# vitasoftAI/ImageRetrievalResearch

Hardware: AMD Instinct MI355X
Metric: images/sec embed + queries/sec top-k@100k-gallery, EffNet-B3a 224^2 (higher is better)
Workload: dtype bf16

## Files before the change

### imageretrievalresearch_amd/_lib.py

```python
from __future__ import annotations

import ctypes as C
import os

_HERE = os.path.dirname(os.path.abspath(__file__))
LIB_PATH = os.environ.get("MI355_LIB_PATH") or os.path.join(_HERE, "libmi355_retrieval.so")

c_f32p = C.POINTER(C.c_float)
c_i64p = C.POINTER(C.c_int64)
vp = C.c_void_p


class GemmExArgs(C.Structure):
    _fields_ = [("A", vp), ("lda", C.c_int), ("W", vp), ("ldw", C.c_int), ("bias", vp),
                ("res", vp), ("ldr", C.c_int), ("res_n", C.c_int),
                ("gate", vp), ("gate_ld", C.c_int), ("rows_per_img", C.c_int), ("a_relu6", C.c_int),
                ("out", vp), ("ldo", C.c_int), ("out_f32", C.c_int),
                ("M", C.c_int), ("N", C.c_int), ("K", C.c_int), ("act", C.c_int),
                ("M_sel", C.c_int64), ("splitk_ws", vp), ("splitk_ws_bytes", C.c_size_t),
                ("ln_stats", vp), ("ln_colsum", vp)]


class RankFilter(C.Structure):
    _fields_ = [("query_labels", vp), ("gallery_labels", vp), ("label_mode", C.c_int), ("exclude", vp)]
# ... 51 lines not shown
    "mi355_model_num_tensors": (C.c_int, [vp]),
    "mi355_model_tensor_info": (C.c_int, [vp, C.c_int, C.POINTER(C.c_char_p), C.POINTER(C.c_int),
                                          C.POINTER(C.c_int64), C.POINTER(C.c_int)]),
    "mi355_model_feature_dim": (C.c_int, [vp]),
    "mi355_model_num_classes": (C.c_int, [vp]),
    "mi355_model_set_tensor": (C.c_int, [vp, C.c_char_p, vp, C.c_int64]),
    "mi355_model_pack": (C.c_int, [vp, vp]),
    "mi355_model_forward_features": (C.c_int, [vp, vp, C.c_int, C.c_int, C.c_int, vp, vp, vp]),
    "mi355_model_forward": (C.c_int, [vp, vp, C.c_int, C.c_int, C.c_int, vp, vp, vp]),
    "mi355_model_forward_u8": (C.c_int, [vp, vp, C.c_int, C.c_int, C.c_int, C.c_int, C.POINTER(C.c_float), C.POINTER(C.c_float),
                                         vp, C.c_int, vp, vp, vp]),
    "mi355_model_enable_taps": (C.c_int, [vp, C.c_int]),
    "mi355_model_read_tap": (C.c_int, [vp, C.c_char_p, vp, C.c_int64, C.POINTER(C.c_int64), vp]),
    "mi355_model_run_between_taps": (C.c_int, [vp, C.c_char_p, C.c_char_p, vp, C.c_int, C.c_int, C.c_int, C.c_int, vp]),
    "mi355_model_traffic": (C.c_int, [vp, C.c_int, C.c_int, C.c_int, C.POINTER(C.c_double),
                                      C.POINTER(C.c_double), C.POINTER(C.c_double)]),
    "mi355_model_traffic_kinds": (C.c_int, [vp, C.c_int, C.c_int, C.c_int, C.POINTER(C.c_double),
                                            C.POINTER(C.c_double), C.c_int]),
    "mi355_model_set_option": (C.c_int, [vp, C.c_char_p, C.c_int64]),
    "mi355_model_profile_read": (C.c_int, [vp, C.POINTER(C.c_double), C.POINTER(C.c_int64), C.c_int]),
    "mi355_model_profile_ops": (C.c_int, [vp, C.c_int, C.c_int, C.c_int, C.c_int, C.POINTER(C.c_double),
                                          C.POINTER(C.c_double), C.POINTER(C.c_int), C.c_char_p, C.c_int]),
    "mi355_model_block_stamps": (C.c_int, [vp, C.POINTER(C.c_double), C.c_int]),
    "mi355_pool_linear": (C.c_int, [vp, C.c_int, C.c_int, C.c_int, vp, vp, C.c_int, vp, vp, vp]),
    "mi355_gemm_bf16": (C.c_int, [vp, vp, vp, vp, C.c_int, C.c_int, C.c_int, C.c_int, C.c_int, vp]),
    "mi355_gemm_bf16_ex": (C.c_int, [vp, C.POINTER(C.c_int), vp]),
    "mi355_window_attention": (C.c_int, [vp, vp, vp, C.c_int, C.c_int, C.c_int, C.c_int, C.c_int, vp]),
    "mi355_square_pad_normalize": (C.c_int, [vp, C.c_int, C.c_int, C.c_int, C.POINTER(C.c_float), C.POINTER(C.c_float), vp, vp]),
    "mi355_conv_input_silu": (C.c_int, [vp, vp, C.c_int, C.c_int, C.c_int, vp, vp]),
    "mi355_resize_bilinear_u8": (C.c_int, [vp, C.c_int, C.c_int, vp, C.c_int, C.c_int, vp, vp]),
    "mi355_resize_batch_workspace_bytes": (C.c_size_t, [vp, C.c_int, C.c_int, C.c_int, C.c_int]),
    "mi355_resize_batch_u8": (C.c_int, [vp, C.c_int64, vp, vp, C.c_int, C.c_int, C.c_int, C.c_int, C.c_int, vp, vp, C.c_size_t,
                                        vp]),
    "mi355_model_forward_images_workspace_bytes": (C.c_size_t, [vp, C.c_int, C.c_int, C.c_int]),
    "mi355_model_forward_images": (C.c_int, [vp, vp, C.c_int64, vp, vp, C.c_int, C.c_int, C.c_int, C.c_int, C.POINTER(C.c_float),
                                             C.POINTER(C.c_float), vp, C.c_int, vp, vp, vp, C.c_size_t, vp]),
    "mi355_score_boost": (C.c_int, [vp, C.c_int64, C.c_float, C.c_float, C.c_float, C.c_int, vp, vp]),
}

_lib = None


class MI355Error(RuntimeError):
    """A libmi355_retrieval call returned nonzero; the message is mi355_last_error()."""


# ... 33 lines not shown
```

### imageretrievalresearch_amd/csrc/mbconv_block.hip

```cpp
#include "ops.h"

namespace mi355 {

typedef __bf16 bf16x8 __attribute__((ext_vector_type(8)));
typedef float f32x4 __attribute__((ext_vector_type(4)));
typedef unsigned u32x4 __attribute__((ext_vector_type(4)));
typedef unsigned u32x2 __attribute__((ext_vector_type(2)));

constexpr int MB_THREADS = 512;
constexpr int MB_WAVES = MB_THREADS / 64;
constexpr int MB_MAX_RD = 192;
constexpr int MB_MC = MB_WAVES * 16;

__device__ __forceinline__ float mb_lo(unsigned u) { return __uint_as_float(u << 16); }
__device__ __forceinline__ float mb_hi(unsigned u) { return __uint_as_float(u & 0xffff0000u); }

__device__ __forceinline__ void mb_lds_barrier() {
    asm volatile("s_waitcnt lgkmcnt(0)" ::: "memory");
    __builtin_amdgcn_s_barrier();
    asm volatile("" ::: "memory");
}

__host__ __device__ static inline int mb_proj_ntw(int NTp, int MTp, int NTW) {
    int best = 1, best_busy = 0;
// ... 12 lines not shown
    const int ntw = mb_proj_ntw(NTp, MTp, 3);
    if (wi != 14) return ntw;
    const int nwn = (NTp + ntw - 1) / ntw;
    int msplit = nwn <= MB_WAVES ? MB_WAVES / nwn : 1;
    if (msplit > MTp) msplit = MTp;
    if (nwn <= MB_WAVES && (MTp + msplit - 1) / msplit <= mwp) return ntw;
    return 4;
}

template <int KS> struct MbTaps {
    static constexpr int KK = KS * KS;
    static constexpr int NV = (KS / 2) * KS;
    static constexpr int NH = (KS + 1) / 2;
    static constexpr int NP = NV + NH;
    __host__ __device__ static constexpr bool vertical(int tp) { return tp < NV; }
    __host__ __device__ static constexpr int tap_a(int tp) {
        return tp < NV ? (tp / KS) * 2 * KS + tp % KS : (KS - 1) * KS + (tp - NV) * 2;
    }
    __host__ __device__ static constexpr int tap_b(int tp) {
        return tp < NV ? tap_a(tp) + KS : ((tp - NV) * 2 + 1 < KS ? tap_a(tp) + 1 : -1);
    }
};

template <int KS, int S, int WI, int MW, int MH, int NTW, int MWP, int KST, int A_IT, int ACT_E, int ACT_D>
__global__ __launch_bounds__(MB_THREADS) void k_mbconv_block(const BlockArgs a) {
    using TP = MbTaps<KS>;
    constexpr int MC = MB_MC;
    constexpr int PAD = KS / 2;
    constexpr int NP = TP::NP;
    constexpr int EW = WI + 2 * PAD;
    constexpr int WO = (WI + 2 * PAD - KS) / S + 1;
    constexpr int TR = WO <= 8 ? 2 : 1;
    constexpr int RP = (TR == 2 && S == 1) ? ((EW + 7) & ~7) : EW;
    static_assert(WO <= 16, "depthwise tile geometry");
    constexpr bool PROJ_WHOLE = WI == 7 && NTW == 2;
    constexpr int KC = WI == 7 ? 256 : 128;
    constexpr int ALD = KC + 16;
    extern __shared__ __attribute__((aligned(16))) unsigned char mb_smem[];

    const int tid = threadIdx.x, lane = tid & 63;
    const int wave = __builtin_amdgcn_readfirstlane(tid >> 6);
    const int fr = lane & 15, fq = lane >> 4, fk = fq * 8;
    const int b = blockIdx.x;
    const int P = a.H * a.W, MT = (P + 15) >> 4, XLD = a.XLD;
    const int EH = a.H + 2 * PAD;
    const int EP = (EH + (TR == 2 ? S : 0)) * RP + 8;
    const int Pout = a.Ho * a.Wo;
    const int MTo = TR == 2 ? (a.Ho + 1) >> 1 : a.Ho;
    const int midp = (a.mid + 15) & ~15;

    bf16_t* Xs = reinterpret_cast<bf16_t*>(mb_smem);
    size_t off = ((size_t)MT * 16 * XLD * 2 + 64 + 15) & ~(size_t)15;
    float* pool = reinterpret_cast<float*>(mb_smem + off);
    off += (size_t)((a.mid + 255) & ~255) * 4;
    float* rvec = reinterpret_cast<float*>(mb_smem + off);
    off += MB_MAX_RD * 4;
    unsigned char* R = mb_smem + off;
    bf16_t* Es = reinterpret_cast<bf16_t*>(R) + (size_t)wave * EP * 16;

    const bool stamping = a.stamps != nullptr;
    unsigned t_acc[8] = {0, 0, 0, 0, 0, 0, 0, 0};
    unsigned t_last = 0;
    if (stamping) t_last = (unsigned)__builtin_readcyclecounter();
    auto tick = [&](int i) {
        if (stamping) { const unsigned t = (unsigned)__builtin_readcyclecounter(); t_acc[i] += t - t_last; t_last = t; }
    };

    const int nslabs = (a.mid + MC - 1) / MC;
    const int rb0 = (a.norot & 1) ? 0 : b, rb1 = (a.norot & 2) ? 0 : b, rb2 = (a.norot & 4) ? 0 : b, rb3 = (a.norot & 8) ? 0 : b;
    auto slab_of = [&](int ci) { return (ci + rb0) % nslabs; };

    u32x4 wq[KST];
    f32x4 be_reg;
    auto w_prefetch_slab = [&](int cbase) {
        const int n = min(cbase + wave * 16 + fr, midp - 1);
#pragma unroll
        for (int h = 0; h < KST; ++h) wq[h] = *reinterpret_cast<const u32x4*>(a.We + (n * a.Kp + fk + h * 32));
        be_reg = *reinterpret_cast<const f32x4*>(a.be + min(cbase + wave * 16 + fq * 4, midp - 4));
        __builtin_amdgcn_sched_barrier(0);
    };
    unsigned short wd_raw[NP], wd_nxt[NP];
    f32x4 bd_reg, bd_nxt;
    auto wd_fetch = [&](int cbase) {
        const int ch = min(cbase + wave * 16 + fr, a.mid - 1);
#pragma unroll
        for (int tp = 0; tp < NP; ++tp) {
            const int ta = TP::tap_a(tp), tb = TP::tap_b(tp) < 0 ? TP::tap_a(tp) : TP::tap_b(tp);
            const int t = (lane & 32) ? tb : ta;
            wd_nxt[tp] = a.Wd[t * a.mid + ch];
        }
        bd_nxt = *reinterpret_cast<const f32x4*>(a.bd + min(cbase + wave * 16 + fq * 4, a.mid - 4));
        __builtin_amdgcn_sched_barrier(0);
// ... 22 lines not shown
            if (id0 == tid) {
                bf16_t* Eall = reinterpret_cast<bf16_t*>(R);
                for (int id = tid; id < MB_WAVES * EP * 2; id += MB_THREADS)
                    *reinterpret_cast<u32x4*>(&Eall[id * 8]) = (u32x4){0u, 0u, 0u, 0u};
                if (tid < 4) *reinterpret_cast<u32x4*>(&Xs[MT * 16 * XLD + tid * 8]) = (u32x4){0u, 0u, 0u, 0u};
            }
#pragma unroll
            for (int u = 0; u < U; ++u)
                if (dst[u] >= 0) *reinterpret_cast<u32x4*>(&Xs[dst[u]]) = v[u];
        }
    }
    mb_lds_barrier();
    tick(0);

    bf16_t* Db = a.D + (size_t)b * Pout * a.mid;

    const int e_cv = (fq & 1) * 8 + ((fq >> 1) ? RP * 16 : 0);
    const int e_ch = (fq & 1) * 8 + ((fq >> 1) ? 16 : 0);
    const int t_row = TR == 2 ? (fr >> 3) : 0, t_col = TR == 2 ? (fr & 7) : fr;
    const int e_lane = (t_row * S * RP + t_col * S) * 16;
    constexpr int E_TILE = TR * S * RP * 16;
    const bool col_ok = t_col < WO;

    const int abl = a.variant;
    bool prev_active = false;
    for (int ci = 0; ci < nslabs; ++ci) {
        const int cbase = slab_of(ci) * MC;
        const int ch0 = cbase + wave * 16;
        const bool active = ch0 < a.mid;
        {
            constexpr int MTO_SQ = TR == 2 ? (WO + 1) / 2 : WO;
            if (ci > 0 && prev_active && MTo == MTO_SQ) {
                if constexpr (MTO_SQ >= 14) asm volatile("s_waitcnt vmcnt(14)" ::: "memory");
                else if constexpr (MTO_SQ >= 4) asm volatile("s_waitcnt vmcnt(4)" ::: "memory");
                else asm volatile("s_waitcnt vmcnt(1)" ::: "memory");
            } else {
                asm volatile("s_waitcnt vmcnt(0)" ::: "memory");
            }
#pragma unroll
            for (int h = 0; h < KST; ++h) asm volatile("" : "+v"(wq[h]));
            asm volatile("" : "+v"(be_reg));
            asm volatile("" : "+v"(bd_nxt));
#pragma unroll
            for (int tp = 0; tp < NP; ++tp) { asm volatile("" : "+v"(wd_nxt[tp])); wd_raw[tp] = wd_nxt[tp]; }
            bd_reg = bd_nxt;
        }
        tick(1);
// ... 468 lines not shown
#pragma unroll
                    for (int j = 0; j < NTW; ++j) {
                        const int n = (wn * ntw + j) * 16 + fq * 4;
                        if (j < ntw && n < a.Cout) {
                            float v[4] = {acc[j][i].x, acc[j][i].y, acc[j][i].z, acc[j][i].w};
                            if (a.has_res && n < a.res_n) {
                                v[0] += mb_lo(rr[j][i].x); v[1] += mb_hi(rr[j][i].x); v[2] += mb_lo(rr[j][i].y); v[3] += mb_hi(rr[j][i].y);
                            }
                            u32x2 o;
                            o.x = pack2bf(v[0], v[1]);
                            o.y = pack2bf(v[2], v[3]);
                            *reinterpret_cast<u32x2*>(Yb + (m * a.Cout + n)) = o;
                        }
                    }
                }
            }
        }
    }
    tick(7);
    if (stamping && tid == 0) {
        long long* o = a.stamps + (size_t)b * 16;
#pragma unroll
        for (int i = 0; i < 8; ++i) o[i] = (long long)t_acc[i];
    }
}

struct MbGeom { int wi, mw, mh, ntw, mwp, a_it; };
static bool mb_geom(int H, int W, MbGeom* g) {
    if (W == 7 && H * W <= 64) { *g = {7, 4, 1, 3, 4, 4}; return true; }
    if (W == 14 && H * W <= 208) { *g = {14, 7, 2, 3, 7, 7}; return true; }
    return false;
}
#define MB_INSTANCES(X)                                                                                              \
    X(3, 1, 14, 3, 3, ACT_SILU) X(5, 1, 14, 3, 3, ACT_SILU) X(5, 1, 14, 5, 3, ACT_SILU) X(5, 2, 14, 5, 2, ACT_SILU)     \
    X(5, 1, 7, 8, 2, ACT_SILU) X(3, 1, 7, 8, 3, ACT_SILU) X(3, 1, 7, 12, 3, ACT_SILU)                                 \
    X(3, 1, 14, 4, 2, ACT_NONE) X(3, 1, 14, 4, 3, ACT_NONE) X(3, 1, 14, 5, 3, ACT_NONE) X(3, 1, 14, 6, 3, ACT_NONE)   \
    X(3, 1, 7, 7, 2, ACT_NONE) X(3, 1, 7, 8, 2, ACT_NONE) X(3, 1, 7, 8, 3, ACT_NONE) X(3, 1, 7, 9, 3, ACT_NONE)       \
    X(3, 1, 7, 10, 3, ACT_NONE) X(3, 1, 7, 11, 3, ACT_NONE) X(3, 1, 14, 6, 4, ACT_NONE)
static bool mb_instance_ok(int k, int stride, int wi, int kst, int ntw, int act_d) {
#define X(KS, S, WI, KST, NTW, AD) if (k == KS && stride == S && wi == WI && kst == KST && ntw == NTW && act_d == AD) return true;
    MB_INSTANCES(X)
#undef X
    return false;
}

static int mb_pick_kcs(const BlockArgs& a) {
// ... 68 lines not shown
    return mb_pick_xld(a, k, g) != 0;
}

template <int KS, int S, int WI, int MW, int MH, int NTW, int MWP, int KST, int A_IT, int ACT_E, int ACT_D>
static int launch_mb(BlockArgs a, int B, hipStream_t st) {
    MbGeom g;
    mb_geom(a.H, a.W, &g);
    a.XLD = mb_pick_xld(a, KS, g);
    a.KCS = mb_pick_kcs(a);
    const size_t lds = mb_lds_bytes_xld(a, KS, a.XLD, g);
    static bool attr_done[64] = {false};
    int dev = 0;
    MI355_CHECK_HIP(hipGetDevice(&dev));
    if (dev >= 0 && dev < 64 && !attr_done[dev]) {
        MI355_CHECK_HIP(hipFuncSetAttribute((const void*)k_mbconv_block<KS, S, WI, MW, MH, NTW, MWP, KST, A_IT, ACT_E, ACT_D>,
                                            hipFuncAttributeMaxDynamicSharedMemorySize, 160 * 1024));
        attr_done[dev] = true;
    }
    hipLaunchKernelGGL((k_mbconv_block<KS, S, WI, MW, MH, NTW, MWP, KST, A_IT, ACT_E, ACT_D>), dim3(B), dim3(MB_THREADS), lds, st, a);
    MI355_LAUNCH_CHECK();
    return OK;
}

int launch_mbconv_block(const BlockArgs& a, int B, int k, int stride, hipStream_t st) {
    MI355_REQUIRE(mbconv_block_supported(a.H, a.W, a.Cin, a.mid, a.Cout, k, stride, a.rd, a.act_e, a.act_d), "mbconv_block: unsupported shape");
    const int Pout = a.Ho * a.Wo;
    MbGeom gg;
    mb_geom(a.H, a.W, &gg);
    const int ntw = mb_pick_ntw((a.Cout + 15) / 16, (Pout + 15) / 16, gg.wi, gg.mwp);
    const int kst = a.Kp / 32;
#define X(KS, S, WI, KST, NTW, AD)                                                                  \
    if (k == KS && stride == S && a.W == WI && kst == KST && ntw == NTW && a.act_d == AD)           \
        return launch_mb<KS, S, WI, (WI == 7 ? 4 : 7), (WI == 7 ? 1 : 2), NTW, (WI == 7 ? 4 : 7), KST, (WI == 7 ? 4 : 7), ACT_SILU, AD>(a, B, st);
    MB_INSTANCES(X)
#undef X
    set_error("mbconv_block: no instance for k=%d s=%d W=%d Kp=%d ntw=%d", k, stride, a.W, a.Kp, ntw);
    return ERR_UNSUPPORTED;
}

}
```

### imageretrievalresearch_amd/csrc/model.hip

```cpp
#include "model_exec.h"
#include "../../include/mi355_retrieval.h"

#include <string.h>

#include <algorithm>

namespace mi355 {

int pack_gemm(Packer& pk, Op& op) {
    const TensorSpec* w = pk.get(op.w_name);
    if (!w) return ERR_STATE;
    const int N = op.cout_real, K = op.cin_real;
    MI355_REQUIRE(w->numel() == (int64_t)N * K, "pack: %s has %lld elements, expected %d x %d", op.w_name.c_str(),
                  (long long)w->numel(), N, K);
    std::vector<float> scale, shift;
    if (!pk.bn_fold(op.bn_name, op.bn_eps, N, scale, shift)) return ERR_STATE;
    if (!op.bias_name.empty()) {
        const TensorSpec* b = pk.get(op.bias_name);
        if (!b) return ERR_STATE;
        for (int i = 0; i < N; ++i) shift[i] = b->data[i] * scale[i] + shift[i];
    }
    const int Np = (op.cout + 15) & ~15, Kp = (op.cin + 31) & ~31;
    op.w_off = pk.alloc((size_t)Np * Kp * 2);
    op.b_off = pk.alloc((size_t)Np * 4);
// ... 318 lines not shown
    if (g.out != SLOT_E || d.in != SLOT_E || d.out != SLOT_D || p.in != SLOT_D || !p.use_gate || !d.pool) return false;
    if (g.use_gate || g.res != SLOT_NONE || g.a_relu6 || !g.tap.empty() || !d.tap.empty()) return false;
    if (p.act != ACT_NONE || (p.res != SLOT_NONE && p.res != g.in)) return false;
    if (p.res != SLOT_NONE && p.res_channels && ((p.res_channels + 7) & ~7) != g.cin) return false;
    return mbconv_block_supported(h, w, g.cin, g.cout, p.cout, d.k, d.stride, s.rd, g.act, d.act);
}

static int stamp_ptr(ExecCtx& cx, size_t oi, long long** out) {
    mi355_model* m = cx.m;
    *out = nullptr;
    if (!m->block_stamps) return OK;
    const size_t need = m->def.ops.size() * (size_t)cx.B * 16 * sizeof(long long);
    if (m->stamp_bytes < need) {
        if (m->stamp_buf) MI355_CHECK_HIP(hipFree(m->stamp_buf));
        MI355_CHECK_HIP(hipMalloc((void**)&m->stamp_buf, need));
        m->stamp_bytes = need;
    }
    m->stamp_B = cx.B;
    *out = m->stamp_buf + (oi * (size_t)cx.B + cx.b0) * 16;
    MI355_CHECK_HIP(hipMemsetAsync(*out, 0, (size_t)cx.nb * 16 * sizeof(long long), cx.st));
    return OK;
}

static int exec_block(ExecCtx& cx, size_t oi) {
    mi355_model* m = cx.m;
    SlotState* S = m->slots;
    const Op& g = m->def.ops[oi];
    const Op& d = m->def.ops[oi + 1];
    const Op& s = m->def.ops[oi + 2];
    const Op& p = m->def.ops[oi + 3];
    BlockArgs a{};
    a.X = (const bf16_t*)cx.slot_ptr(g.in);
    a.We = (const bf16_t*)cx.w(g.w_off); a.be = (const float*)cx.w(g.b_off);
    a.Wd = (const bf16_t*)cx.w(d.w_off); a.bd = (const float*)cx.w(d.b_off);
    a.W1 = (const bf16_t*)cx.w(s.w3_off); a.b1 = (const float*)cx.w(s.b_off);
    a.W2 = (const bf16_t*)cx.w(s.w4_off); a.b2 = (const float*)cx.w(s.b2_off);
    a.Wp = (const bf16_t*)cx.w(p.w_off); a.bp = (const float*)cx.w(p.b_off);
    a.D = (bf16_t*)cx.slot_ptr(d.out);
    a.Y = (bf16_t*)cx.slot_ptr(p.out);
    a.H = S[g.in].h; a.W = S[g.in].w; a.Cin = g.cin; a.Kp = (g.cin + 31) & ~31; a.mid = g.cout;
    a.Ho = S[d.out].h; a.Wo = S[d.out].w; a.Cout = p.cout; a.Kp2 = (p.cin + 31) & ~31; a.rd = s.rd;
    a.has_res = p.res != SLOT_NONE;
    a.res_n = p.res != SLOT_NONE ? (p.res_channels ? ((p.res_channels + 7) & ~7) : p.cout) : 0;
    a.a_relu6 = p.a_relu6;
    a.act_e = g.act; a.act_d = d.act; a.se_act = s.se_act;
    a.inv_hw = 1.0f / (float)(a.Ho * a.Wo);
    a.norot = m->block_norot;
    a.variant = m->block_variant;
    a.stamps = nullptr;
    { const int rc = stamp_ptr(cx, oi, &a.stamps); if (rc != OK) return rc; }
    return launch_mbconv_block(a, cx.nb, d.k, d.stride, cx.st);
}

static int exec_fused(ExecCtx& cx, const Op& g, const Op& d) {
    mi355_model* m = cx.m;
    SlotState* S = m->slots;
    FusedArgs a{};
    a.X = (const bf16_t*)cx.slot_ptr(g.in);
    a.We = (const bf16_t*)cx.w(g.w_off); a.be = (const float*)cx.w(g.b_off);
    a.Wd = (const bf16_t*)cx.w(d.w_off); a.bd = (const float*)cx.w(d.b_off);
    a.D = (bf16_t*)cx.slot_ptr(d.out);
    a.pool = d.pool ? (float*)cx.slot_ptr(SLOT_POOLPART) : nullptr;
    a.H = S[g.in].h; a.W = S[g.in].w; a.Cin = g.cin; a.Kp = (g.cin + 31) & ~31; a.mid = g.cout;
    a.Ho = S[d.out].h; a.Wo = S[d.out].w; a.act_e = g.act; a.act_d = d.act;
    a.debug_skip = m->fuse_debug;
    if (fused_late_supported(a.H, a.W, g.cin, g.cout, d.k, d.stride)) {
        m->pool_nblk = 1;
        return launch_fused_late(a, cx.nb, d.k, d.stride, cx.st);
    }
    if (use_sweep(m, g, d, a.H, a.W)) {
        SweepArgs sa{};
        sa.X = a.X; sa.We = a.We; sa.be = a.be; sa.Wd = a.Wd; sa.bd = a.bd; sa.D = a.D; sa.pool = a.pool;
        sa.H = a.H; sa.W = a.W; sa.Cin = a.Cin; sa.Kp = a.Kp; sa.mid = a.mid; sa.Ho = a.Ho; sa.Wo = a.Wo;
        sa.act_e = a.act_e; sa.act_d = a.act_d; sa.csplit_override = m->sweep_csplit; sa.variant = m->sweep_variant; sa.debug_skip = m->sweep_skip;
// ... 34 lines not shown
            S[d.out].c = d.cout;
            if (block) {
                const Op& pj = m->def.ops[oi + 3];
                S[pj.out].h = S[d.out].h; S[pj.out].w = S[d.out].w; S[pj.out].c = pj.cout;
            }
        } else
        switch (op.kind) {
            case OP_STEM: S[op.out].h = conv_out(cx.H, 3, 2); S[op.out].w = conv_out(cx.W, 3, 2); S[op.out].c = op.cout; break;
            case OP_GEMM: S[op.out].h = S[op.in].h; S[op.out].w = S[op.in].w; S[op.out].c = op.cout; break;
            case OP_DW: {
                const int ho = conv_out(S[op.in].h, op.k, op.stride), wo = conv_out(S[op.in].w, op.k, op.stride);
                S[op.out].h = ho; S[op.out].w = wo; S[op.out].c = op.cout;
                break;
            }
            case OP_SE: break;
            default: if (op.out != SLOT_NONE) { S[op.out].h = op.tokens_h; S[op.out].w = op.tokens_h; S[op.out].c = op.cout; } break;
        }
        hipEvent_t e0 = nullptr, e1 = nullptr;
        if (m->profile) {
            MI355_CHECK_HIP(hipEventCreate(&e0));
            MI355_CHECK_HIP(hipEventCreate(&e1));
            MI355_CHECK_HIP(hipEventRecord(e0, cx.st));
        }
        {
            char lab[192] = "";
            if (roctx_active())
                op_range_label(op, cx.H, cx.W, in_h, in_w, block ? "block: " : (fused ? "fused: " : ""), lab, sizeof lab);
            RoctxRange range(lab);
            if (block) {
                if (int e = exec_block(cx, oi)) return e;
            } else if (fused) {
                if (int e = exec_fused(cx, op, m->def.ops[oi + 1])) return e;
            } else if (int e = exec_op(cx, op)) return e;
        }
        if (m->profile) {
            MI355_CHECK_HIP(hipEventRecord(e1, cx.st));
            m->prof_events.push_back({op_index, {e0, e1}});
            if (m->prof_fused.size() < m->def.ops.size()) m->prof_fused.resize(m->def.ops.size(), 0);
            m->prof_fused[op_index] = fused ? 1 : 0;
        }
        if (block) {
            const Op& pj = m->def.ops[oi + 3];
            if (m->taps && !pj.tap.empty())
                if (int e = record_tap(cx, pj)) return e;
            oi += 3;
            continue;
        }
        if (m->taps && !op.tap.empty())
            if (int e = record_tap(cx, op)) return e;
        if (fused) ++oi;
    }
    return OK;
}

struct U8Source {
    const unsigned char* img = nullptr;
    const int64_t* desc = nullptr;
    int h = 0, w = 0, fill = 255;
    float mean[3] = {0.f, 0.f, 0.f}, stdv[3] = {1.f, 1.f, 1.f};
    const float* conv_w = nullptr;
};

static int forward_impl(mi355_model* m, const float* x, int B, int H, int W, float* out, float* pooled_out,
                        bool features_only, hipStream_t st, const U8Source* u8 = nullptr) {
    MI355_REQUIRE(m, "forward: null model");
    MI355_REQUIRE(m->packed, "forward: weights not packed (call mi355_model_pack after set_tensor)");
    MI355_REQUIRE((x || u8) && out, "forward: null input/output pointer");
    MI355_REQUIRE(B >= 1 && H >= 32 && W >= 32, "forward: bad shape B=%d H=%d W=%d", B, H, W);
// ... 331 lines not shown
    MI355_REQUIRE(it != m->tapbufs.end(), "read_tap: no tap named '%s' was recorded", tap_name);
    const TapBuf& t = it->second;
    if (shape) { shape[0] = t.B; shape[1] = t.c_real; shape[2] = t.h; shape[3] = t.w; }
    if (!out) return OK;
    MI355_REQUIRE(out_numel >= (int64_t)t.B * t.c_real * t.h * t.w, "read_tap: output too small");
    return launch_nhwc_to_nchw_f32((const bf16_t*)t.ptr, out, t.B, t.h * t.w, t.c, t.c_real, (hipStream_t)stream);
}

int mi355_model_set_option(mi355_model_t m, const char* key, int64_t value) {
    MI355_REQUIRE(m && key, "set_option: null argument");
    const std::string k = key;
    if (k == "microbatch") m->microbatch = (int)value;
    else if (k == "lanes") m->lanes = (int)value;
    else if (k == "fuse") m->fuse = value != 0;
    else if (k == "fuse_band") m->fuse_band = (int)value;
    else if (k == "fuse_sweep") m->fuse_sweep = (int)value;
    else if (k == "sweep_csplit") m->sweep_csplit = (int)value;
    else if (k == "sweep_variant") m->sweep_variant = (int)value;
    else if (k == "sweep_skip") m->sweep_skip = (int)value;
    else if (k == "fuse_debug") m->fuse_debug = (int)value;
    else if (k == "fuse_ln") m->fuse_ln = (int)value;
    else if (k == "fuse_block") m->fuse_block = (int)value;
    else if (k == "fuse_block_min_batch") m->fuse_block_min_batch = (int)value;
    else if (k == "block_stamps") m->block_stamps = value != 0;
    else if (k == "block_norot") m->block_norot = (int)value;
    else if (k == "block_variant") m->block_variant = (int)value;
    else if (k == "fuse_head_gap") m->fuse_head_gap = value != 0;
    else if (k == "roctx") roctx_enable(value != 0);
    else if (k == "profile") {
        m->profile = value != 0;
        for (int i = 0; i < PK_COUNT; ++i) { m->prof_ms[i] = 0; m->prof_launches[i] = 0; }
        m->prof_op_ms.assign(m->def.ops.size(), 0.0);
        m->prof_op_n.assign(m->def.ops.size(), 0);
    } else {
        set_error("set_option: unknown option '%s'", key);
        return ERR_ARG;
    }
    return OK;
}

int mi355_model_profile_read(mi355_model_t m, double* ms_by_kind, int64_t* launches_by_kind, int n) {
    MI355_REQUIRE(m && ms_by_kind && launches_by_kind && n >= PK_COUNT, "profile_read: need arrays of >= %d", PK_COUNT);
    for (auto& pe : m->prof_events) {
        MI355_CHECK_HIP(hipEventSynchronize(pe.second.second));
        float ms = 0.f;
        MI355_CHECK_HIP(hipEventElapsedTime(&ms, pe.second.first, pe.second.second));
// ... 106 lines not shown
                if (op.out != SLOT_NONE) { S[op.out].h = op.tokens_h; S[op.out].w = op.tokens_h; }
                const double t = (double)op.tokens_h * op.tokens_h;
                if (op.kind == OP_PATCH_EMBED) bytes_by_kind[kd] += (double)B * (3.0 * H * W * 4 + t * op.cout_real * 2);
                else if (op.kind == OP_TOKEN_MEAN) bytes_by_kind[kd] += B * t * op.cin_real * 2;
                else bytes_by_kind[kd] += B * t * (op.cin_real + op.cout_real) * 2;
                if (op.kind == OP_WINATTN) macs_by_kind[kd] += B * t * 49.0 * op.cout_real * 2;
                if (op.kind == OP_PATCH_EMBED) macs_by_kind[kd] += B * t * 48.0 * op.cout_real;
                break;
            }
        }
    }
    return OK;
}

int mi355_model_traffic(mi355_model_t m, int B, int H, int W, double* act_bytes, double* weight_bytes, double* macs) {
    MI355_REQUIRE(m, "traffic: null model");
    double by[PK_COUNT], mc[PK_COUNT];
    if (int e = mi355_model_traffic_kinds(m, B, H, W, by, mc, PK_COUNT)) return e;
    double tb = 0, tm = 0;
    for (int i = 0; i < PK_COUNT; ++i) { tb += by[i]; tm += mc[i]; }
    if (act_bytes) *act_bytes = tb;
    if (macs) *macs = tm;
    if (weight_bytes) *weight_bytes = (double)m->blob.size();
    return OK;
}

int mi355_model_block_stamps(mi355_model_t m, double* out, int max_ops) {
    MI355_REQUIRE(m && out, "block_stamps: null argument");
    const int n = (int)m->def.ops.size();
    MI355_REQUIRE(max_ops >= n, "block_stamps: need room for %d ops", n);
    for (int i = 0; i < n * 16; ++i) out[i] = 0.0;
    if (!m->stamp_buf || m->stamp_B <= 0) return n;
    MI355_CHECK_HIP(hipDeviceSynchronize());
    std::vector<long long> h((size_t)n * m->stamp_B * 16);
    MI355_CHECK_HIP(hipMemcpy(h.data(), m->stamp_buf, h.size() * sizeof(long long), hipMemcpyDeviceToHost));
    for (int i = 0; i < n; ++i)
        for (int b = 0; b < m->stamp_B; ++b)
            for (int j = 0; j < 16; ++j) out[i * 16 + j] += (double)h[((size_t)i * m->stamp_B + b) * 16 + j] / m->stamp_B;
    return n;
}

static int gemm_zero_page(const bf16_t** zeros) {
    static void* zero_page[MI355_MAX_DEVICES] = {nullptr};
    int dev = 0;
    MI355_CHECK_HIP(hipGetDevice(&dev));
    MI355_REQUIRE(dev >= 0 && dev < MI355_MAX_DEVICES, "gemm_bf16: device ordinal %d out of range", dev);
// ... 81 lines not shown
```

### imageretrievalresearch_amd/csrc/model_exec.h

```cpp
#pragma once
#include "model.h"

#include <string.h>

namespace mi355 {

int swin_exec(const ModelDef& def, const Op& op, struct ExecCtx& cx);

static inline uint16_t f2bf_host(float f) {
    uint32_t u;
    memcpy(&u, &f, 4);
    if ((u & 0x7fffffffu) > 0x7f800000u) return (uint16_t)((u >> 16) | 0x40);
    u += 0x7fffu + ((u >> 16) & 1u);
    return (uint16_t)(u >> 16);
}
static inline float bf_round_host(float f) {
    uint32_t u = ((uint32_t)f2bf_host(f)) << 16;
    float r;
    memcpy(&r, &u, 4);
    return r;
}

struct SlotState {
    size_t off = 0, bytes = 0;
// ... 14 lines not shown

struct mi355_model {
    ModelDef def;
    std::vector<char> blob;
    void* dev_blob = nullptr;
    size_t dev_blob_bytes = 0;
    bool packed = false;
    void* arena = nullptr;
    size_t arena_bytes = 0;
    int arena_device = -1, blob_device = -1;
    SlotState slots[SLOT_COUNT];
    int microbatch = 0;
    int lanes = 1;
    hipStream_t lane_stream[4] = {nullptr, nullptr, nullptr, nullptr};
    hipEvent_t lane_fork = nullptr, lane_join[4] = {nullptr, nullptr, nullptr, nullptr};
    size_t lane_bytes = 0;
    int fuse_sweep = 1;
    int sweep_variant = 0, sweep_skip = 0;
    int sweep_csplit = 0;
    int fuse_band = 2;
    bool fuse = true;
    int fuse_block = 1;
    int fuse_block_min_batch = 96;
    bool fuse_head_gap = true;
    int block_variant = 0;
    int block_norot = 0;
    bool block_stamps = false;
    long long* stamp_buf = nullptr; size_t stamp_bytes = 0; int stamp_B = 0;
    int fuse_debug = 0;
    int fuse_ln = 1;
    int pool_nblk = 0;
    bool taps = false;
    std::map<std::string, TapBuf> tapbufs;
    bool profile = false;
    std::vector<std::pair<int, std::pair<hipEvent_t, hipEvent_t>>> prof_events;
    std::vector<char> prof_fused;
    std::vector<double> prof_op_ms;
    std::vector<long> prof_op_n;
    double prof_ms[PK_COUNT] = {0};
    long prof_launches[PK_COUNT] = {0};
};

namespace mi355 {

struct ExecCtx {
    mi355_model* m;
// ... 51 lines not shown
```

### imageretrievalresearch_amd/csrc/ops.h

```cpp
#pragma once
#include "common.h"

namespace mi355 {

struct GemmArgs {
    const bf16_t* A; int lda;
    const bf16_t* W; int ldw;
    const float* bias;
    const bf16_t* res; int ldr; int res_n;
    const float* gate; int gate_ld; int rows_per_img;
    void* out; int ldo; int out_f32;
    int M, N, K;
    int act;
    int a_relu6;
    const bf16_t* zeros;
    long M_sel;
    float* splitk_ws;
    size_t splitk_ws_bytes;
    const float* ln_stats;
    const float* ln_colsum;
};
int launch_gemm_bf16(const GemmArgs& a, hipStream_t st, int* path = nullptr);
bool gemm_wide_supported(const GemmArgs& a);
int launch_gemm_wide(const GemmArgs& a, hipStream_t st);
// ... 40 lines not shown
struct BlockArgs {
    const bf16_t* X;
    const bf16_t* We; const float* be;
    const bf16_t* Wd; const float* bd;
    const bf16_t* W1; const float* b1;
    const bf16_t* W2; const float* b2;
    const bf16_t* Wp; const float* bp;
    bf16_t* D;
    bf16_t* Y;
    long long* stamps;
    int H, W, Cin, Kp, mid, Ho, Wo, Cout, Kp2, rd;
    int XLD;
    int KCS;
    int norot;
    int variant;
    int has_res;
    int res_n;
    int a_relu6;
    int act_e, act_d, se_act;
    float inv_hw;
};
bool mbconv_block_supported(int H, int W, int Cin, int mid, int Cout, int k, int stride, int rd, int act_e, int act_d);
int launch_mbconv_block(const BlockArgs& a, int B, int k, int stride, hipStream_t st);

int launch_stem(const float* x, const float* w, const float* bias, bf16_t* out, int B, int H, int W, int Cout,
                int act, hipStream_t st);

int launch_stem_u8(const unsigned char* img, int h, int w, int fill, const float* mean, const float* stdv,
                   const float* conv_w, const float* sw, const float* bias, bf16_t* out, int B, int Cout, int act,
                   hipStream_t st, const int64_t* desc = nullptr, int b0 = 0);

int check_images(const unsigned char* pixels, int64_t pixels_bytes, const int64_t* desc_host, const int64_t* desc_dev, int B,
                 const char* who);
size_t resize_batch_workspace(const int64_t* desc_host, int B, int out_h, int out_w, bool pad);
int resize_batch(const unsigned char* pixels, int64_t pixels_bytes, const int64_t* desc_host, const int64_t* desc_dev, int B,
                 int out_h, int out_w, bool pad, int fill, unsigned char* out, void* workspace, size_t workspace_bytes,
                 hipStream_t st);

int dw_pool_blocks(int Ho, int Wo, int C);
int launch_dwconv(const bf16_t* in, const bf16_t* w, const float* bias, bf16_t* out, float* pool_partial, int B,
                  int H, int W, int C, int k, int stride, int act, int* pool_nblk, hipStream_t st);

int launch_se(const float* pool_partial, int nblk, float inv_hw, const float* w1, const float* b1, const float* w2,
              const float* b2, float* gate, int B, int C, int rd, int act1, hipStream_t st);

int launch_gap(const bf16_t* in, float* pooled, bf16_t* pooled_bf16, int B, int HW, int C, hipStream_t st);
// ... 17 lines not shown
```

### imageretrievalresearch_amd/models.py

```python
from __future__ import annotations

import ctypes as C
import math
import operator
import weakref

import torch
import torch.nn as nn

from ._lib import MI355Error, check, lib, require_cuda, stream_ptr

_FAMILY = {
    "efficientnet_b3a": "efficientnet", "efficientnet_b3": "efficientnet",
    "rexnet_100": "rexnet", "rexnet_130": "rexnet", "rexnet_150": "rexnet", "rexnet_200": "rexnet",
    "swin_base_patch4_window7_224": "swin",
}
_HEAD_PATH = {"efficientnet": "classifier", "rexnet": "head.fc", "swin": "head"}


_VERSION_OF = operator.attrgetter("_version")


def list_models():
    return sorted(_FAMILY)
# ... 250 lines not shown
        self.__dict__["_dirty"] = False
        self.__dict__["_pack_device"] = device
        self.__dict__["_sig_tensors"] = None
        self.__dict__["_sig"] = self._signature()

    def _ensure_packed(self, device):
        if self._dirty or self._pack_device != device or self._sig != self._signature():
            self._pack(device)

    def set_option(self, key: str, value: int):
        check(lib().mi355_model_set_option(self._handle, key.encode(), int(value)))
        return self

    def traffic(self, B: int, H: int = 224, W: int = 224):
        a, w, m = C.c_double(), C.c_double(), C.c_double()
        check(lib().mi355_model_traffic(self._handle, B, H, W, C.byref(a), C.byref(w), C.byref(m)))
        by = (C.c_double * 8)()
        mc = (C.c_double * 8)()
        check(lib().mi355_model_traffic_kinds(self._handle, B, H, W, by, mc, 8))
        kinds = ["stem", "gemm", "dw", "se", "other", "attn", "ln", "fused"]
        return {"act_bytes": a.value, "weight_bytes": w.value, "macs": m.value,
                "bytes_by_kind": dict(zip(kinds, list(by))), "macs_by_kind": dict(zip(kinds, list(mc)))}

    def profile_read(self):
        ms = (C.c_double * 8)()
        n = (C.c_int64 * 8)()
        check(lib().mi355_model_profile_read(self._handle, ms, n, 8))
        kinds = ["stem", "gemm", "dw", "se", "other", "attn", "ln", "fused"]
        return {k: {"ms": ms[i], "launches": n[i]} for i, k in enumerate(kinds)}

    def profile_ops(self, B: int, H: int = 224, W: int = 224):
        n = 1024
        ms = (C.c_double * n)()
        by = (C.c_double * n)()
        kd = (C.c_int * n)()
        lab = C.create_string_buffer(n * 64)
        cnt = lib().mi355_model_profile_ops(self._handle, B, H, W, n, ms, by, kd, lab, 64)
        kinds = ["stem", "gemm", "dw", "se", "other", "attn", "ln", "fused"]
        return [(lab.raw[i * 64:(i + 1) * 64].split(b"\0")[0].decode(), kinds[kd[i]], ms[i], by[i]) for i in range(cnt)]

    def block_stamps(self):
        n = 1024
        out = (C.c_double * (n * 16))()
        cnt = lib().mi355_model_block_stamps(self._handle, out, n)
        if cnt < 0:
            check(1)
# ... 209 lines not shown
```

### include/mi355_retrieval.h

```cpp
#ifndef MI355_RETRIEVAL_H
#define MI355_RETRIEVAL_H

#include <stddef.h>
#include <stdint.h>

#ifdef __cplusplus
extern "C" {
#endif

#define MI355_ABI_VERSION 3

int mi355_abi_version(void);
const char* mi355_last_error(void);
int mi355_device_count(void);

int mi355_synth_fill(float* out, int64_t n, uint64_t seed, int64_t offset, int kind, void* stream);


int mi355_l2_normalize_rows(const float* in, float* out, int64_t rows, int dim, float eps, void* stream);

size_t mi355_rank_workspace_bytes(int64_t Q, int64_t G, int dim, int k);

int mi355_rank_topk(const float* queries, int64_t Q, const float* gallery, int64_t G, int dim,
                    int gallery_is_normalized, int k, float eps, int64_t idx_offset,
// ... 127 lines not shown
                               const float* stdv, const float* conv_input_w, int features_only, float* out, float* pooled_out,
                               void* workspace, size_t workspace_bytes, void* stream);

int mi355_model_enable_taps(mi355_model_t m, int enable);
int mi355_model_read_tap(mi355_model_t m, const char* tap_name, float* out, int64_t out_numel,
                         int64_t shape[4], void* stream);

int mi355_model_run_between_taps(mi355_model_t m, const char* from_tap, const char* to_tap, const float* x, int B,
                                 int C, int h, int w, void* stream);

int mi355_model_traffic(mi355_model_t m, int B, int H, int W, double* act_bytes, double* weight_bytes,
                        double* macs);

int mi355_model_traffic_kinds(mi355_model_t m, int B, int H, int W, double* bytes_by_kind, double* macs_by_kind, int n);

int mi355_model_set_option(mi355_model_t m, const char* key, int64_t value);
int mi355_model_profile_read(mi355_model_t m, double* ms_by_kind, int64_t* launches_by_kind, int n);

int mi355_model_profile_ops(mi355_model_t m, int B, int H, int W, int max_ops, double* avg_ms, double* bytes,
                            int* kinds, char* labels, int label_stride);

int mi355_model_block_stamps(mi355_model_t m, double* out, int max_ops);

int mi355_pool_linear(const float* fm, int B, int C, int HW, const float* weight, const float* bias, int N, float* out,
                      float* pooled_out, void* stream);

int mi355_gemm_bf16(const void* A, const void* W, const float* bias, void* out, int M, int N, int K, int ldw, int act,
                    void* stream);

typedef struct mi355_gemm_ex_args {
    const void* A; int lda;
    const void* W; int ldw;
    const float* bias;
    const void* res; int ldr; int res_n;
    const float* gate; int gate_ld; int rows_per_img; int a_relu6;
    void* out; int ldo; int out_f32;
    int M, N, K, act;
    int64_t M_sel;
    void* splitk_ws; size_t splitk_ws_bytes;
    const float* ln_stats; const float* ln_colsum;
} mi355_gemm_ex_args;

enum {
    MI355_GEMM_PATH_TILE_M64_BK32 = 1,
    MI355_GEMM_PATH_TILE_M64_BK64 = 2,
    MI355_GEMM_PATH_TILE = 3,
// ... 35 lines not shown
```

Measured before the change: 62510.

## Chain consecutive same-shape MBConv blocks into one persistent kernel launch

Adds a k_mbconv_chain kernel that runs up to five consecutive identical-shape MBConv blocks in a single launch, with each workgroup processing its image through every block and synchronising with __syncthreads between them. The per-block body is factored into a device function with a DIAG template flag, so the diagnostic paths (stamps, norot, variant) are compiled out of the chained variant. The aim is to cut kernel launch overhead and inter-kernel gaps for the 14x14 and 7x7 stages. The cost is extra template instances and large kernel arguments. Correctness relies on each workgroup owning a whole image, so the next block only reads that workgroup's own prior output.

```diff
diff --git a/imageretrievalresearch_amd/_lib.py b/imageretrievalresearch_amd/_lib.py
--- a/imageretrievalresearch_amd/_lib.py
+++ b/imageretrievalresearch_amd/_lib.py
@@ -97,6 +97,7 @@
     "mi355_model_profile_ops": (C.c_int, [vp, C.c_int, C.c_int, C.c_int, C.c_int, C.POINTER(C.c_double),
                                           C.POINTER(C.c_double), C.POINTER(C.c_int), C.c_char_p, C.c_int]),
     "mi355_model_block_stamps": (C.c_int, [vp, C.POINTER(C.c_double), C.c_int]),
+    "mi355_model_launch_counts": (C.c_int, [vp, C.POINTER(C.c_int64)]),
     "mi355_pool_linear": (C.c_int, [vp, C.c_int, C.c_int, C.c_int, vp, vp, C.c_int, vp, vp, vp]),
     "mi355_gemm_bf16": (C.c_int, [vp, vp, vp, vp, C.c_int, C.c_int, C.c_int, C.c_int, C.c_int, vp]),
     "mi355_gemm_bf16_ex": (C.c_int, [vp, C.POINTER(C.c_int), vp]),
diff --git a/imageretrievalresearch_amd/csrc/mbconv_block.hip b/imageretrievalresearch_amd/csrc/mbconv_block.hip
--- a/imageretrievalresearch_amd/csrc/mbconv_block.hip
+++ b/imageretrievalresearch_amd/csrc/mbconv_block.hip
@@ -58,8 +58,8 @@
     }
 };
 
-template <int KS, int S, int WI, int MW, int MH, int NTW, int MWP, int KST, int A_IT, int ACT_E, int ACT_D>
-__global__ __launch_bounds__(MB_THREADS) void k_mbconv_block(const BlockArgs a) {
+template <int KS, int S, int WI, int MW, int MH, int NTW, int MWP, int KST, int A_IT, int ACT_E, int ACT_D, bool DIAG>
+__device__ __forceinline__ void mb_block_body(const BlockArgs& a, const int tid, const int b) {
     using TP = MbTaps<KS>;
     constexpr int MC = MB_MC;
     constexpr int PAD = KS / 2;
@@ -74,10 +74,9 @@
     constexpr int ALD = KC + 16;
     extern __shared__ __attribute__((aligned(16))) unsigned char mb_smem[];
 
-    const int tid = threadIdx.x, lane = tid & 63;
+    const int lane = tid & 63;
     const int wave = __builtin_amdgcn_readfirstlane(tid >> 6);
     const int fr = lane & 15, fq = lane >> 4, fk = fq * 8;
-    const int b = blockIdx.x;
     const int P = a.H * a.W, MT = (P + 15) >> 4, XLD = a.XLD;
     const int EH = a.H + 2 * PAD;
     const int EP = (EH + (TR == 2 ? S : 0)) * RP + 8;
@@ -94,7 +93,7 @@
     unsigned char* R = mb_smem + off;
     bf16_t* Es = reinterpret_cast<bf16_t*>(R) + (size_t)wave * EP * 16;
 
-    const bool stamping = a.stamps != nullptr;
+    const bool stamping = DIAG && a.stamps != nullptr;
     unsigned t_acc[8] = {0, 0, 0, 0, 0, 0, 0, 0};
     unsigned t_last = 0;
     if (stamping) t_last = (unsigned)__builtin_readcyclecounter();
@@ -103,7 +102,8 @@
     };
 
     const int nslabs = (a.mid + MC - 1) / MC;
-    const int rb0 = (a.norot & 1) ? 0 : b, rb1 = (a.norot & 2) ? 0 : b, rb2 = (a.norot & 4) ? 0 : b, rb3 = (a.norot & 8) ? 0 : b;
+    const int norot = DIAG ? a.norot : 0;
+    const int rb0 = (norot & 1) ? 0 : b, rb1 = (norot & 2) ? 0 : b, rb2 = (norot & 4) ? 0 : b, rb3 = (norot & 8) ? 0 : b;
     auto slab_of = [&](int ci) { return (ci + rb0) % nslabs; };
 
     u32x4 wq[KST];
@@ -172,7 +172,7 @@
     constexpr int E_TILE = TR * S * RP * 16;
     const bool col_ok = t_col < WO;
 
-    const int abl = a.variant;
+    const int abl = DIAG ? a.variant : 0;
     bool prev_active = false;
     for (int ci = 0; ci < nslabs; ++ci) {
         const int cbase = slab_of(ci) * MC;
@@ -687,6 +687,31 @@
         long long* o = a.stamps + (size_t)b * 16;
 #pragma unroll
         for (int i = 0; i < 8; ++i) o[i] = (long long)t_acc[i];
+    }
+}
+
+template <int KS, int S, int WI, int MW, int MH, int NTW, int MWP, int KST, int A_IT, int ACT_E, int ACT_D>
+__global__ __launch_bounds__(MB_THREADS) void k_mbconv_block(const BlockArgs a) {
+    mb_block_body<KS, S, WI, MW, MH, NTW, MWP, KST, A_IT, ACT_E, ACT_D, true>(a, threadIdx.x, blockIdx.x);
+}
+
+constexpr int MB_CHAIN_MAX = MBCONV_CHAIN_MAX;
+struct ChainArgs {
+    BlockArgs blk[MB_CHAIN_MAX];
+    int n;
+};
+
+template <int KS, int S, int WI, int MW, int MH, int NTW, int MWP, int KST, int A_IT, int ACT_E, int ACT_D>
+__global__ __launch_bounds__(MB_THREADS) void k_mbconv_chain(const ChainArgs c) {
+#pragma unroll
+    for (int i = 0; i < MB_CHAIN_MAX; ++i) {
+        if (i >= c.n) break;
+        if (i > 0) __syncthreads();
+        int tid = threadIdx.x, b = blockIdx.x, bi = i;
+        asm volatile("" : "+v"(tid));
+        asm volatile("" : "+s"(b));
+        if constexpr (WI == 14) asm volatile("" : "+s"(bi));
+        mb_block_body<KS, S, WI, MW, MH, NTW, MWP, KST, A_IT, ACT_E, ACT_D, false>(c.blk[bi], tid, b);
     }
 }
 
@@ -801,6 +826,69 @@
     return OK;
 }
 
+#define MB_CHAIN_INSTANCES(X) X(3, 1, 14, 3, 3, ACT_SILU) X(5, 1, 14, 5, 3, ACT_SILU) X(5, 1, 7, 8, 2, ACT_SILU)
+
+static int mb_ntw_of(const BlockArgs& a) {
+    MbGeom gg;
+    mb_geom(a.H, a.W, &gg);
+    return mb_pick_ntw((a.Cout + 15) / 16, (a.Ho * a.Wo + 15) / 16, gg.wi, gg.mwp);
+}
+
+bool mbconv_chain_supported(const BlockArgs& a, int k, int stride) {
+    if (!mbconv_block_supported(a.H, a.W, a.Cin, a.mid, a.Cout, k, stride, a.rd, a.act_e, a.act_d)) return false;
+    const int kst = a.Kp / 32, ntw = mb_ntw_of(a);
+#define X(KS, S, WI, KST, NTW, AD) if (k == KS && stride == S && a.W == WI && kst == KST && ntw == NTW && a.act_d == AD) return true;
+    MB_CHAIN_INSTANCES(X)
+#undef X
+    return false;
+}
+
+template <int KS, int S, int WI, int MW, int MH, int NTW, int MWP, int KST, int A_IT, int ACT_E, int ACT_D>
+static int launch_chain(const BlockArgs* a, int n, int B, hipStream_t st) {
+    MbGeom g;
+    mb_geom(a[0].H, a[0].W, &g);
+    ChainArgs c{};
+    c.n = n;
+    for (int i = 0; i < n; ++i) {
+        c.blk[i] = a[i];
+        c.blk[i].XLD = mb_pick_xld(a[i], KS, g);
+        c.blk[i].KCS = mb_pick_kcs(a[i]);
+        MI355_REQUIRE(c.blk[i].XLD == c.blk[0].XLD && c.blk[i].KCS == c.blk[0].KCS, "mbconv_chain: blocks of different geometry");
+    }
+    const size_t lds = mb_lds_bytes_xld(c.blk[0], KS, c.blk[0].XLD, g);
+    static bool attr_done[64] = {false};
+    int dev = 0;
+    MI355_CHECK_HIP(hipGetDevice(&dev));
+    if (dev >= 0 && dev < 64 && !attr_done[dev]) {
+        MI355_CHECK_HIP(hipFuncSetAttribute((const void*)k_mbconv_chain<KS, S, WI, MW, MH, NTW, MWP, KST, A_IT, ACT_E, ACT_D>,
+                                            hipFuncAttributeMaxDynamicSharedMemorySize, 160 * 1024));
+        attr_done[dev] = true;
+    }
+    hipLaunchKernelGGL((k_mbconv_chain<KS, S, WI, MW, MH, NTW, MWP, KST, A_IT, ACT_E, ACT_D>), dim3(B), dim3(MB_THREADS), lds, st, c);
+    MI355_LAUNCH_CHECK();
+    return OK;
+}
+
+int launch_mbconv_chain(const BlockArgs* a, int n, int B, int k, int stride, hipStream_t st) {
+    MI355_REQUIRE(a && n >= 1 && n <= MB_CHAIN_MAX, "mbconv_chain: %d blocks (1..%d)", n, MB_CHAIN_MAX);
+    MI355_REQUIRE(mbconv_chain_supported(a[0], k, stride), "mbconv_chain: unsupported shape");
+    for (int i = 1; i < n; ++i) {
+        const BlockArgs &p = a[0], &q = a[i];
+        MI355_REQUIRE(q.H == p.H && q.W == p.W && q.Cin == p.Cin && q.Kp == p.Kp && q.mid == p.mid && q.Ho == p.Ho && q.Wo == p.Wo &&
+                      q.Cout == p.Cout && q.Kp2 == p.Kp2 && q.rd == p.rd && q.act_e == p.act_e && q.act_d == p.act_d,
+                      "mbconv_chain: block %d differs in shape from block 0", i);
+        MI355_REQUIRE(q.X == a[i - 1].Y, "mbconv_chain: block %d does not read block %d's output", i, i - 1);
+    }
+    const int kst = a[0].Kp / 32, ntw = mb_ntw_of(a[0]);
+#define X(KS, S, WI, KST, NTW, AD)                                                                  \
+    if (k == KS && stride == S && a[0].W == WI && kst == KST && ntw == NTW && a[0].act_d == AD)     \
+        return launch_chain<KS, S, WI, (WI == 7 ? 4 : 7), (WI == 7 ? 1 : 2), NTW, (WI == 7 ? 4 : 7), KST, (WI == 7 ? 4 : 7), ACT_SILU, AD>(a, n, B, st);
+    MB_CHAIN_INSTANCES(X)
+#undef X
+    set_error("mbconv_chain: no instance for k=%d s=%d W=%d Kp=%d ntw=%d", k, stride, a[0].W, a[0].Kp, ntw);
+    return ERR_UNSUPPORTED;
+}
+
 int launch_mbconv_block(const BlockArgs& a, int B, int k, int stride, hipStream_t st) {
     MI355_REQUIRE(mbconv_block_supported(a.H, a.W, a.Cin, a.mid, a.Cout, k, stride, a.rd, a.act_e, a.act_d), "mbconv_block: unsupported shape");
     const int Pout = a.Ho * a.Wo;
diff --git a/imageretrievalresearch_amd/csrc/model.hip b/imageretrievalresearch_amd/csrc/model.hip
--- a/imageretrievalresearch_amd/csrc/model.hip
+++ b/imageretrievalresearch_amd/csrc/model.hip
@@ -364,14 +364,14 @@
     return OK;
 }
 
-static int exec_block(ExecCtx& cx, size_t oi) {
+static void block_args(ExecCtx& cx, size_t oi, BlockArgs& a) {
     mi355_model* m = cx.m;
     SlotState* S = m->slots;
     const Op& g = m->def.ops[oi];
     const Op& d = m->def.ops[oi + 1];
     const Op& s = m->def.ops[oi + 2];
     const Op& p = m->def.ops[oi + 3];
-    BlockArgs a{};
+    a = BlockArgs{};
     a.X = (const bf16_t*)cx.slot_ptr(g.in);
     a.We = (const bf16_t*)cx.w(g.w_off); a.be = (const float*)cx.w(g.b_off);
     a.Wd = (const bf16_t*)cx.w(d.w_off); a.bd = (const float*)cx.w(d.b_off);
@@ -390,8 +390,53 @@
     a.norot = m->block_norot;
     a.variant = m->block_variant;
     a.stamps = nullptr;
+}
+
+static int exec_block(ExecCtx& cx, size_t oi) {
+    BlockArgs a;
+    block_args(cx, oi, a);
     { const int rc = stamp_ptr(cx, oi, &a.stamps); if (rc != OK) return rc; }
+    cx.m->block_launches++;
+    const Op& d = cx.m->def.ops[oi + 1];
     return launch_mbconv_block(a, cx.nb, d.k, d.stride, cx.st);
+}
+
+static int chain_length(ExecCtx& cx, size_t oi, size_t op_end) {
+    mi355_model* m = cx.m;
+    if (!m->fuse_chain || m->profile || m->taps || m->block_stamps || m->block_variant || m->block_norot) return 1;
+    const std::vector<Op>& ops = m->def.ops;
+    BlockArgs a0;
+    block_args(cx, oi, a0);
+    const Op& d0 = ops[oi + 1];
+    if (a0.Ho != a0.H || a0.Wo != a0.W || !mbconv_chain_supported(a0, d0.k, d0.stride)) return 1;
+    int n = 1;
+    for (size_t j = oi + 4; n < MBCONV_CHAIN_MAX && j + 3 < op_end; j += 4, ++n) {
+        const Op &g = ops[j], &d = ops[j + 1], &s = ops[j + 2], &p = ops[j + 3], &prev = ops[j - 1];
+        if (g.in != prev.out || !can_fuse_block(m, j, a0.H, a0.W, cx.B)) break;
+        if (g.cin != ops[oi].cin || g.cout != ops[oi].cout || p.cout != ops[oi + 3].cout || p.cin != ops[oi + 3].cin ||
+            d.k != d0.k || d.stride != d0.stride || s.rd != ops[oi + 2].rd || g.act != ops[oi].act || d.act != d0.act ||
+            s.se_act != ops[oi + 2].se_act || p.a_relu6 != ops[oi + 3].a_relu6 || (p.res != SLOT_NONE) != (ops[oi + 3].res != SLOT_NONE) ||
+            p.res_channels != ops[oi + 3].res_channels)
+            break;
+        if (p.out == g.in || d.out != d0.out || p.out == d0.out) break;
+    }
+    return n;
+}
+
+static int exec_chain(ExecCtx& cx, size_t oi, int n) {
+    mi355_model* m = cx.m;
+    SlotState* S = m->slots;
+    const std::vector<Op>& ops = m->def.ops;
+    BlockArgs a[MBCONV_CHAIN_MAX];
+    block_args(cx, oi, a[0]);
+    for (int i = 1; i < n; ++i) {
+        const size_t j = oi + 4 * (size_t)i;
+        S[ops[j + 3].out].h = S[ops[oi + 3].out].h; S[ops[j + 3].out].w = S[ops[oi + 3].out].w; S[ops[j + 3].out].c = ops[j + 3].cout;
+        block_args(cx, j, a[i]);
+    }
+    m->chain_launches++;
+    const Op& d = m->def.ops[oi + 1];
+    return launch_mbconv_chain(a, n, cx.nb, d.k, d.stride, cx.st);
 }
 
 static int exec_fused(ExecCtx& cx, const Op& g, const Op& d) {
@@ -472,12 +517,21 @@
             MI355_CHECK_HIP(hipEventCreate(&e1));
             MI355_CHECK_HIP(hipEventRecord(e0, cx.st));
         }
+        const int chain = block ? chain_length(cx, oi, op_end) : 1;
         {
             char lab[192] = "";
-            if (roctx_active())
-                op_range_label(op, cx.H, cx.W, in_h, in_w, block ? "block: " : (fused ? "fused: " : ""), lab, sizeof lab);
+            if (roctx_active()) {
+                if (chain > 1) {
+                    const Op &d = m->def.ops[oi + 1], &pj = m->def.ops[oi + 3];
+                    snprintf(lab, sizeof lab, "embed/chain: %d blocks (ops %zu-%zu) %d->%d->%d k%d @%dx%d", chain, oi, oi + 4 * (size_t)chain - 1,
+                             op.cin_real, op.cout_real, pj.cout_real, d.k, in_h, in_w);
+                } else
+                    op_range_label(op, cx.H, cx.W, in_h, in_w, block ? "block: " : (fused ? "fused: " : ""), lab, sizeof lab);
+            }
             RoctxRange range(lab);
-            if (block) {
+            if (chain > 1) {
+                if (int e = exec_chain(cx, oi, chain)) return e;
+            } else if (block) {
                 if (int e = exec_block(cx, oi)) return e;
             } else if (fused) {
                 if (int e = exec_fused(cx, op, m->def.ops[oi + 1])) return e;
@@ -493,7 +547,7 @@
             const Op& pj = m->def.ops[oi + 3];
             if (m->taps && !pj.tap.empty())
                 if (int e = record_tap(cx, pj)) return e;
-            oi += 3;
+            oi += 3 + 4 * (size_t)(chain - 1);
             continue;
         }
         if (m->taps && !op.tap.empty())
@@ -871,6 +925,7 @@
     else if (k == "fuse_ln") m->fuse_ln = (int)value;
     else if (k == "fuse_block") m->fuse_block = (int)value;
     else if (k == "fuse_block_min_batch") m->fuse_block_min_batch = (int)value;
+    else if (k == "fuse_chain") m->fuse_chain = (int)value;
     else if (k == "block_stamps") m->block_stamps = value != 0;
     else if (k == "block_norot") m->block_norot = (int)value;
     else if (k == "block_variant") m->block_variant = (int)value;
@@ -1023,6 +1078,13 @@
     if (act_bytes) *act_bytes = tb;
     if (macs) *macs = tm;
     if (weight_bytes) *weight_bytes = (double)m->blob.size();
+    return OK;
+}
+
+int mi355_model_launch_counts(mi355_model_t m, int64_t* counts) {
+    MI355_REQUIRE(m && counts, "launch_counts: null argument");
+    counts[0] = m->block_launches;
+    counts[1] = m->chain_launches;
     return OK;
 }
 
diff --git a/imageretrievalresearch_amd/csrc/model_exec.h b/imageretrievalresearch_amd/csrc/model_exec.h
--- a/imageretrievalresearch_amd/csrc/model_exec.h
+++ b/imageretrievalresearch_amd/csrc/model_exec.h
@@ -60,6 +60,8 @@
     bool fuse = true;
     int fuse_block = 1;
     int fuse_block_min_batch = 96;
+    int fuse_chain = 1;
+    long long block_launches = 0, chain_launches = 0;
     bool fuse_head_gap = true;
     int block_variant = 0;
     int block_norot = 0;
diff --git a/imageretrievalresearch_amd/csrc/ops.h b/imageretrievalresearch_amd/csrc/ops.h
--- a/imageretrievalresearch_amd/csrc/ops.h
+++ b/imageretrievalresearch_amd/csrc/ops.h
@@ -86,6 +86,9 @@
 };
 bool mbconv_block_supported(int H, int W, int Cin, int mid, int Cout, int k, int stride, int rd, int act_e, int act_d);
 int launch_mbconv_block(const BlockArgs& a, int B, int k, int stride, hipStream_t st);
+constexpr int MBCONV_CHAIN_MAX = 5;
+bool mbconv_chain_supported(const BlockArgs& a, int k, int stride);
+int launch_mbconv_chain(const BlockArgs* a, int n, int B, int k, int stride, hipStream_t st);
 
 int launch_stem(const float* x, const float* w, const float* bias, bf16_t* out, int B, int H, int W, int Cout,
                 int act, hipStream_t st);
diff --git a/imageretrievalresearch_amd/models.py b/imageretrievalresearch_amd/models.py
--- a/imageretrievalresearch_amd/models.py
+++ b/imageretrievalresearch_amd/models.py
@@ -296,6 +296,11 @@
         return {"act_bytes": a.value, "weight_bytes": w.value, "macs": m.value,
                 "bytes_by_kind": dict(zip(kinds, list(by))), "macs_by_kind": dict(zip(kinds, list(mc)))}
 
+    def launch_counts(self):
+        n = (C.c_int64 * 2)()
+        check(lib().mi355_model_launch_counts(self._handle, n))
+        return {"block": n[0], "chain": n[1]}
+
     def profile_read(self):
         ms = (C.c_double * 8)()
         n = (C.c_int64 * 8)()
diff --git a/include/mi355_retrieval.h b/include/mi355_retrieval.h
--- a/include/mi355_retrieval.h
+++ b/include/mi355_retrieval.h
@@ -173,6 +173,8 @@
 
 int mi355_model_block_stamps(mi355_model_t m, double* out, int max_ops);
 
+int mi355_model_launch_counts(mi355_model_t m, int64_t* counts);
+
 int mi355_pool_linear(const float* fm, int B, int C, int HW, const float* weight, const float* bias, int N, float* out,
                       float* pooled_out, void* stream);
 
```

New measurement: 62960 (median of 6 runs). No clear change (+0.7%).
